# EndlessReform/smoltts

Measured on AMD Instinct MI355X. Metric: Mimi frames/sec (=12.5 x RTF), greedy DualAR decode + Mimi decode to PCM, higher is better.
Workload: dtype bf16 weights, fp32 activations/accumulate, fp32 KV cache (LM); fp32 (Mimi)

## Files before the change

include/smoltts_hip.h:

```cpp
#ifndef SMOLTTS_HIP_H
#define SMOLTTS_HIP_H

#include <stddef.h>
#include <stdint.h>

#ifdef __cplusplus
extern "C" {
#endif

#define SMOLTTS_ABI_VERSION 8

enum {
  SMOLTTS_OK = 0,
  SMOLTTS_E_INVALID = -1,
  SMOLTTS_E_HIP = -2,
  SMOLTTS_E_STATE = -3,
  SMOLTTS_E_CAPACITY = -4
};

const char* smoltts_last_error(void);
int smoltts_abi_version(void);



typedef struct SmolttsBlockWeights {
// ... 200 lines not shown

int smoltts_mimi_create(const SmolttsMimiConfig* cfg, const SmolttsMimiWeights* offsets,
                        const void* arena_dev, size_t arena_bytes, SmolttsMimi** out);
void smoltts_mimi_destroy(SmolttsMimi* m);

size_t smoltts_mimi_slab_bytes(const SmolttsMimi* m, int32_t max_batch, int32_t max_chunk_frames);
int smoltts_mimi_session_create(SmolttsMimi* m, void* slab_dev, size_t slab_bytes, int32_t max_batch,
                                int32_t max_chunk_frames, SmolttsMimiSession** out);
void smoltts_mimi_session_destroy(SmolttsMimiSession* s);
int smoltts_mimi_reset(SmolttsMimiSession* s, void* stream);

int smoltts_mimi_reset_slots(SmolttsMimiSession* s, const int32_t* slots_host, int32_t n_slots, void* stream);

#define SMOLTTS_MIMI_OPT_STATELESS_UPSAMPLE 1
#define SMOLTTS_MIMI_OPT_PRODUCTS 2
int smoltts_mimi_session_set_option(SmolttsMimiSession* s, int32_t option, int32_t value);

int smoltts_mimi_decode_chunk(SmolttsMimiSession* s, const int32_t* codes_dev, int64_t codes_stride,
                              int32_t frame_stride, int32_t code_offset, int32_t batch,
                              int32_t n_frames, float* pcm_dev, int64_t pcm_stride, void* stream);

typedef struct SmolttsMimiEncConfig {
  int32_t num_codebooks;
  int32_t n_layers;
  int32_t window;
  int32_t max_positions;
  int32_t extra_right;
} SmolttsMimiEncConfig;

typedef struct SmolttsMimiEncWeights {
// ... 323 lines not shown
                                   const SmolttsSlotFilters* filters_dev, const int32_t* frames_dev, const int32_t* history_dev,
                                   const int32_t* history_len_dev, int32_t step, int32_t* ids_dev, void* stream);

int smoltts_k_layernorm(const float* x_dev, const float* w_dev, const float* b_dev, int32_t n_rows,
                        int32_t dim, float eps, float* out_dev, void* stream);

int smoltts_k_seanet_resblock(int32_t channels, int32_t batch, int32_t n_rows, const float* x_dev, int64_t x_bstride,
                              const void* w2_w3_dev, const float* b2_dev, const void* w3_w3_dev, const float* b3_dev, float* out_dev,
                              int64_t o_bstride, int32_t b3_products, void* stream);

int smoltts_k_seanet_last(int32_t batch, int32_t n_rows, const float* in_dev, int64_t in_bstride, const void* wt_w3_dev,
                          const float* bt_dev, const void* w2_w3_dev, const float* b2_dev, const void* w3_w3_dev, const float* b3_dev,
                          const float* final_w_dev, float final_b, float* pcm_dev, int64_t pcm_stride, const int32_t* slot_pos_dev,
                          int32_t b3_products, void* stream);

int smoltts_k_rvq_upsample(const int32_t* codes_dev, int64_t codes_stride, int32_t frame_stride, int32_t code_offset, int32_t nq,
                           int32_t batch, int32_t n_frames, const float* table_dev, const float* upw_dev, const float* carry_in_dev,
                           float* carry_out_dev, float* tx_dev, void* stream);

#ifdef __cplusplus
}
#endif
#endif
```

smoltts_amd/abi.py:

```python
from __future__ import annotations

import ctypes as C
import os
import sys
from pathlib import Path
from typing import List, Optional

LIB_PATH = Path(__file__).resolve().parent / "csrc" / "libsmoltts_hip.so"


class SmolttsError(RuntimeError):
    pass


ABI_VERSION = 8
OK, E_INVALID, E_HIP, E_STATE, E_CAPACITY = 0, -1, -2, -3, -4
MAX_LAYERS, MAX_FAST_LAYERS, MIMI_MAX_LAYERS = 64, 16, 16
KV_F32, KV_BF16 = 0, 1
W_BF16, W_FP8 = 0, 1
OPT_QKV_TABLE, OPT_COMMIT_PICKS, OPT_SPLIT_ATTN, OPT_STREAM_W, OPT_FUSE_DEPTH_ATTN, OPT_FUSE_PICK, OPT_FP8_PREFILL = 1, 2, 3, 4, 5, 6, 7
MIMI_OPT_STATELESS_UPSAMPLE, MIMI_OPT_PRODUCTS = 1, 2
PRO_NONE, PRO_RMSNORM, PRO_ELU, PRO_LAYERNORM = 0, 1, 2, 3
EPI_STORE, EPI_RESID, EPI_SWIGLU, EPI_GELU, EPI_SCALE_RESID, EPI_QKV_ROPE = range(6)
RESAMPLE_OFF, RESAMPLE_S16, RESAMPLE_ULAW = 0, 1, 2
SEAM_FIRST, SEAM_FINAL, SEAM_OFF = 1, 2, 4
FLAC_OFF, FLAC_F32, FLAC_S16 = 0, 1, 2
FILTER_MAX_WINDOW, FILTER_MAX_PENALTY = 64, 1000.0
PREFIX_MAGIC, PREFIX_MAX_INSTALL = 0x58464250, 16

KV_FORMATS = {"fp32": KV_F32, "bf16": KV_BF16}


class BlockWeights(C.Structure):
    _fields_ = [(n, C.c_uint64) for n in ("attn_norm", "wqkv", "wo", "ffn_norm", "w13", "w2")]


# ... 210 lines not shown
    "smoltts_gemm3_attn_fusable": (INT, "i i i"),
    "smoltts_k_gemm3": (INT, "Gemm3Args* p"),
    "smoltts_k_x3_pack": (INT, "p q i i p p p p p p"),
    "smoltts_k_attention": (INT, "p p p p p i i i i i p p p"),
    "smoltts_k_attention_kv": (INT, "p p p p p i i i i i p p i p"),
    "smoltts_k_attention_split": (INT, "p p p p p i i i i i p p i p p p"),
    "smoltts_k_attention_rows3": (INT, "p p p p p i i i i i p i p"),
    "smoltts_k_embed": (INT, "p i i p p i i i i i i p p"),
    "smoltts_k_argmax": (INT, "p i i q p i p p"),
    "smoltts_k_sample": (INT, "p i i q f f Q i i p p"),
    "smoltts_k_sample_rows": (INT, "p i i q p p i p p"),
    "smoltts_k_sample_rows_filtered": (INT, "p i i q p p p p p i p p"),
    "smoltts_k_layernorm": (INT, "p p p i i f p p"),
    "smoltts_k_seanet_resblock": (INT, "i i i p q p p p p p q i p"),
    "smoltts_k_seanet_last": (INT, "i i p q p p p p p p p f p q p i p"),
    "smoltts_k_rvq_upsample": (INT, "p q i i i i i p p p p p p"),
}
DEBUG_HOOKS = {
    "smoltts_profile_begin": (INT, "i i i i"),
    "smoltts_profile_end": (INT, "f* i*"),
}


def _argtype(kind: str):
    if kind.endswith("*"):
        return C.POINTER(_KINDS.get(kind[:-1]) or globals()[kind[:-1]])
    return _KINDS[kind]


def _bind(lib, table) -> None:
# ... 40 lines not shown
```

smoltts_amd/build.py:

```python
from __future__ import annotations

import hashlib
import os
import shutil
import subprocess
import sys
from concurrent.futures import ThreadPoolExecutor
from pathlib import Path
from typing import Optional, Sequence

CSRC = Path(__file__).resolve().parent / "csrc"
LIB = CSRC / "libsmoltts_hip.so"
SOURCES = ["api.hip", "gemm.hip", "gemm_b3.hip", "gemm3.hip", "attention.hip", "small_ops.hip", "lm_engine.hip", "mimi_engine.hip", "mimi_encoder.hip",
           "seanet.hip", "seanet_last.hip", "conv_xs.hip", "conv_ks.hip", "resample.hip", "tsm.hip", "flac.hip", "seam.hip", "trim.hip", "loudness.hip",
           "watermark.hip"]
ARCH = "gfx950"
PRODUCT_FLAGS = [f"--offload-arch={ARCH}", "-O3", "-fPIC", "-std=c++17", "-Wno-unused-result", "-mllvm", "-amdgpu-kernarg-preload-count=16"]
NAMED_VARIANTS = {"hooks": ["-DSMOLTTS_DEBUG_HOOKS"],
                  "knobs": ["-DSMOLTTS_DBG_KNOBS"],
                  "lds_poison": ["-DSMOLTTS_DBG_LDS_POISON"]}


def _hipcc() -> str:
    for cand in (os.environ.get("HIPCC"), "/opt/rocm/bin/hipcc", shutil.which("hipcc")):
        if cand and Path(cand).exists():
            return cand
    raise RuntimeError("hipcc not found (looked at $HIPCC, /opt/rocm/bin/hipcc, PATH)")


# ... 68 lines not shown
```

smoltts_amd/csrc/api.hip:

```cpp
#include <stdarg.h>

#include "common.h"
#include "mimi_common.h"

namespace smoltts {
static thread_local char g_err[1024] = "";

void set_error(const char* fmt, ...) {
  va_list ap;
  va_start(ap, fmt);
  vsnprintf(g_err, sizeof(g_err), fmt, ap);
  va_end(ap);
}
}

using namespace smoltts;

extern "C" {

const char* smoltts_last_error(void) { return g_err; }
int smoltts_abi_version(void) { return SMOLTTS_ABI_VERSION; }

int smoltts_k_gemm(const SmolttsGemmArgs* a, void* stream) {
  ST_REQUIRE(a, SMOLTTS_E_INVALID, "k_gemm: null args");
// ... 93 lines not shown
                          const float* final_w_dev, float final_b, float* pcm_dev, int64_t pcm_stride, const int32_t* slot_pos_dev,
                          int32_t b3_products, void* stream) {
  ST_REQUIRE(pcm_stride >= 4 * (int64_t)n_rows, SMOLTTS_E_INVALID, "k_seanet_last: pcm_stride %lld < 4 * %d rows", (long long)pcm_stride,
             n_rows);
  MimiLastStageArgs a;
  memset(&a, 0, sizeof(a));
  a.batch = batch; a.T = n_rows;
  a.in = in_dev; a.in_bstride = in_bstride;
  a.wt = wt_w3_dev; a.bt = bt_dev; a.w2 = w2_w3_dev; a.b2 = b2_dev; a.w3 = w3_w3_dev; a.b3 = b3_dev;
  a.final_w = final_w_dev; a.final_b = final_b;
  a.pcm = pcm_dev; a.pcm_stride = pcm_stride;
  a.slot_pos = slot_pos_dev; a.b3_products = b3_products;
  return launch_seanet_last(a, (hipStream_t)stream);
}

int smoltts_k_rvq_upsample(const int32_t* codes_dev, int64_t codes_stride, int32_t frame_stride, int32_t code_offset, int32_t nq,
                           int32_t batch, int32_t n_frames, const float* table_dev, const float* upw_dev, const float* carry_in_dev,
                           float* carry_out_dev, float* tx_dev, void* stream) {
  return launch_rvq_upsample(codes_dev, codes_stride, frame_stride, code_offset, nq, batch, n_frames, table_dev, upw_dev, carry_in_dev,
                             carry_out_dev, tx_dev, (hipStream_t)stream);
}

}
```

smoltts_amd/csrc/mimi_common.h:

```cpp
#pragma once
#include "common.h"

namespace smoltts {

constexpr int MIMI_D = 512, MIMI_HEADS = 8, MIMI_FF = 2048;

struct MimiTransformerBufs {
  float *tx, *tn, *tq, *ta, *th;
  float *kc, *vc;
  size_t layer_stride;
  const int *row_pos, *row_slot;
  float* tws = nullptr;
  char *kc3 = nullptr, *vc3 = nullptr;
  size_t layer_stride3 = 0;
  int b3_products = 6;
};

int run_mimi_transformer(const char* arena, const SmolttsMimiLayerWeights* layers, int n_layers, const float* rope,
                         int cache_len, int window, const MimiTransformerBufs& b, int rows, int rows_per_slot,
                         float* last_out, int64_t last_bstride, hipStream_t st);

int launch_mimi_rows(int n_rows, int rows_per_slot, int pos0, int* row_pos, int* row_slot, hipStream_t st,
                     const int* slot_pos = nullptr);

// ... 8 lines not shown
int launch_seanet_resblock(const MimiResblockArgs& a, hipStream_t st);

struct MimiLastStageArgs {
  int batch, T;
  const float* in; int64_t in_bstride;
  const void* wt; const float* bt;
  const void* w2; const float* b2;
  const void* w3; const float* b3;
  const float* final_w; float final_b;
  float* pcm; int64_t pcm_stride;
  const int* slot_pos;
  int b3_products;
};
int launch_seanet_last(const MimiLastStageArgs& a, hipStream_t st);

int launch_rvq_upsample(const int* codes, int64_t codes_stride, int frame_stride, int code_offset, int nq, int batch, int n_frames,
                        const float* table, const float* upw, const float* carry_in, float* carry_out, float* tx, hipStream_t st);

inline SmolttsGemmArgs mimi_gemm_f32(const void* w, const float* x, long ldx, int M, int N, int K, const void* w3 = nullptr) {
  SmolttsGemmArgs a;
  memset(&a, 0, sizeof(a));
  a.w_dev = w; a.w_is_fp32 = 1; a.x_dev = x; a.ldx = ldx; a.M = M; a.N = N; a.K = K;
  a.w3_dev = w3;
  return a;
}

}
```

smoltts_amd/csrc/mimi_engine.hip:

```cpp
#include <stdlib.h>
#include <string.h>

#include <new>

#include "mimi_common.h"

using namespace smoltts;

namespace {
constexpr int D = MIMI_D, HEADS = MIMI_HEADS, FF = MIMI_FF, NCONV = 14, NBUF = 14;
constexpr int SAMPLES = 1920;
constexpr int BUF_C[NBUF] = {512, 1024, 512, 256, 512, 256, 128, 256, 128, 64, 128, 64, 32, 64};
constexpr int BUF_HALO[NBUF] = {6, 1, 2, 0, 1, 2, 0, 1, 2, 0, 2, 0, 0, 0};
constexpr bool FUSED_BLOCK[NCONV] = {false, false, false, false, false, false, false, false, true, false, false, false, false, false};
constexpr int LAST_STAGE = 10;
constexpr bool buf_used(int i) { return i <= LAST_STAGE && !(i >= 1 && FUSED_BLOCK[i - 1]); }
constexpr int BUF_RPF[NBUF] = {2, 2, 16, 16, 16, 96, 96, 96, 480, 480, 480, 1920, 1920, 1920};
}

struct SmolttsMimi {
  SmolttsMimiConfig cfg;
  SmolttsMimiWeights w;
  const char* arena;
  size_t arena_bytes;
};

struct SmolttsMimiSession {
  SmolttsMimi* m;
  int B, chunk;
  float* carry[2];
// ... 2 lines not shown
  float *kc, *vc;
  char *kc3, *vc3;
  size_t kv3_layer;
  int *row_pos, *row_slot;
  float* buf[NBUF];
  size_t buf_bstride[NBUF];
  size_t halo_total;
  char* zero_begin;
  size_t zero_bytes;
  int* pos_dev;
  float final_bias;
  int* pos_host;
  int parity;
  int products;
  int stateless_upsample;
};

namespace {

size_t carve(SmolttsMimiSession* s, char* base) {
  Carver cv{base, 0};
  const size_t B = s->B, F = s->chunk, R = B * 2 * F;
  const SmolttsMimiConfig& c = s->m->cfg;
  const size_t z0 = cv.off;
  s->carry[0] = cv.take<float>(B * D);
  s->carry[1] = cv.take<float>(B * D);
  s->pos_dev = cv.take<int>(B);
  for (int i = 0; i < NBUF; ++i) {
    s->buf_bstride[i] = buf_used(i) ? (size_t)(BUF_HALO[i] + BUF_RPF[i] * F) * BUF_C[i] : 0;
    s->buf[i] = cv.take<float>(B * s->buf_bstride[i]);
// ... 189 lines not shown
  tmp.B = max_batch; tmp.chunk = max_chunk_frames;
  return carve(&tmp, nullptr);
}

int smoltts_mimi_session_create(SmolttsMimi* m, void* slab_dev, size_t slab_bytes, int32_t max_batch,
                                int32_t max_chunk_frames, SmolttsMimiSession** out) {
  ST_REQUIRE(m && slab_dev && out && max_batch > 0 && max_chunk_frames > 0, SMOLTTS_E_INVALID, "mimi_session_create: bad argument");
  ST_REQUIRE(((uintptr_t)slab_dev & 255) == 0, SMOLTTS_E_INVALID, "mimi_session_create: slab must be 256-byte aligned");
  ST_REQUIRE(2 * max_chunk_frames <= m->cfg.max_positions, SMOLTTS_E_CAPACITY, "mimi_session_create: chunk exceeds max_positions");
  const size_t need = smoltts_mimi_slab_bytes(m, max_batch, max_chunk_frames);
  ST_REQUIRE(slab_bytes >= need, SMOLTTS_E_CAPACITY, "mimi_session_create: slab has %zu bytes, %zu needed", slab_bytes, need);
  SmolttsMimiSession* s = new (std::nothrow) SmolttsMimiSession;
  ST_REQUIRE(s, SMOLTTS_E_INVALID, "mimi_session_create: out of host memory");
  memset(s, 0, sizeof(*s));
  s->m = m; s->B = max_batch; s->chunk = max_chunk_frames;
  carve(s, (char*)slab_dev);
  s->pos_host = static_cast<int*>(calloc((size_t)max_batch, sizeof(int)));
  if (s->pos_host == nullptr || hipMemset(s->zero_begin, 0, s->zero_bytes) != hipSuccess ||
      (s->kc3 && (hipMemset(s->kc3, 0, s->kv3_layer * m->cfg.n_layers) != hipSuccess || hipMemset(s->vc3, 0, s->kv3_layer * m->cfg.n_layers) != hipSuccess)) ||
      hipMemcpy(&s->final_bias, m->arena + m->w.convs[NCONV - 1].b, sizeof(float), hipMemcpyDeviceToHost) != hipSuccess) {
    free(s->pos_host);
    delete s;
    set_error("mimi_session_create: allocation or hipMemset failed");
    return SMOLTTS_E_HIP;
  }
  *out = s;
  return SMOLTTS_OK;
}

void smoltts_mimi_session_destroy(SmolttsMimiSession* s) {
// ... 3 lines not shown
}

int smoltts_mimi_reset(SmolttsMimiSession* s, void* stream) {
  ST_REQUIRE(s, SMOLTTS_E_INVALID, "mimi_reset: null session");
  ST_CHECK_HIP(hipMemsetAsync(s->zero_begin, 0, s->zero_bytes, (hipStream_t)stream));
  for (int b = 0; b < s->B; ++b) s->pos_host[b] = 0;
  s->parity = 0;
  return SMOLTTS_OK;
}

int smoltts_mimi_session_set_option(SmolttsMimiSession* s, int32_t option, int32_t value) {
  ST_REQUIRE(s, SMOLTTS_E_INVALID, "mimi_session_set_option: null session");
  if (option == SMOLTTS_MIMI_OPT_PRODUCTS) {
    ST_REQUIRE(value == 3 || value == 6, SMOLTTS_E_INVALID, "mimi_session_set_option: products %d (3 or 6)", value);
    s->products = value;
    return SMOLTTS_OK;
  }
  ST_REQUIRE(option == SMOLTTS_MIMI_OPT_STATELESS_UPSAMPLE, SMOLTTS_E_INVALID, "mimi_session_set_option: unknown option %d", option);
  ST_REQUIRE(value == 0 || value == 1, SMOLTTS_E_INVALID, "mimi_session_set_option: value %d (0 or 1)", value);
  s->stateless_upsample = value;
  return SMOLTTS_OK;
}

int smoltts_mimi_reset_slots(SmolttsMimiSession* s, const int32_t* slots_host, int32_t n_slots, void* stream) {
  ST_REQUIRE(s && slots_host && n_slots > 0, SMOLTTS_E_INVALID, "mimi_reset_slots: bad argument");
  hipStream_t st = (hipStream_t)stream;
  for (int i = 0; i < n_slots; ++i) {
    const int b = slots_host[i];
    ST_TRY(check_slot("mimi_reset_slots", b, s->B));
    ST_CHECK_HIP(hipMemsetAsync(s->carry[0] + (size_t)b * D, 0, D * sizeof(float), st));
// ... 65 lines not shown
    if (i == LAST_STAGE) {
      const SmolttsMimiConv &c2 = m->w.convs[i + 1], &c3 = m->w.convs[i + 2];
      ST_REQUIRE(cv.w3 && c2.w3 && c3.w3 && m->w.final_w && cv.cin == 128 && cv.cout == 64 && cv.stride == 4, SMOLTTS_E_INVALID,
                 "mimi: the arena lacks the W3 tiles of the last stage (or its shape is not 128 -> 64, stride 4)");
      MimiLastStageArgs a;
      memset(&a, 0, sizeof(a));
      a.batch = batch; a.T = BUF_RPF[i] * F;
      a.in = s->buf[i] + (size_t)BUF_HALO[i] * BUF_C[i]; a.in_bstride = (int64_t)s->buf_bstride[i];
      a.wt = A + cv.w3; a.bt = (const float*)(A + cv.b);
      a.w2 = A + c2.w3; a.b2 = (const float*)(A + c2.b); a.w3 = A + c3.w3; a.b3 = (const float*)(A + c3.b);
      a.final_w = (const float*)(A + m->w.final_w); a.final_b = s->final_bias; a.pcm = pcm_dev; a.pcm_stride = pcm_stride;
      a.slot_pos = s->pos_dev; a.b3_products = s->products;
      ST_TRY(launch_seanet_last(a, st));
      break;
    }
    if (FUSED_BLOCK[i]) {
      const SmolttsMimiConv& c1 = m->w.convs[i + 1];
      ST_REQUIRE(cv.w3 && c1.w3, SMOLTTS_E_INVALID, "mimi: the arena lacks the W3 tiles of conv %d", i);
      MimiResblockArgs a;
      memset(&a, 0, sizeof(a));
      a.channels = cv.cin; a.batch = batch; a.T = BUF_RPF[i] * F;
      a.x = s->buf[i] + (size_t)BUF_HALO[i] * BUF_C[i]; a.x_bstride = (int64_t)s->buf_bstride[i];
      a.w2 = A + cv.w3; a.b2 = (const float*)(A + cv.b); a.w3 = A + c1.w3; a.b3 = (const float*)(A + c1.b);
      a.out = s->buf[i + 2] + (size_t)BUF_HALO[i + 2] * BUF_C[i + 2]; a.o_bstride = (int64_t)s->buf_bstride[i + 2];
      a.b3_products = s->products;
      ST_TRY(launch_seanet_resblock(a, st));
      i += 1;
      continue;
    }
    const int Tin = BUF_RPF[i] * F;
// ... 43 lines not shown
```

smoltts_amd/mimi.py:

```python
from __future__ import annotations

import ctypes as C
from typing import Dict, Optional, Sequence

import torch

from . import packing
from .abi import (MIMI_OPT_PRODUCTS, MIMI_OPT_STATELESS_UPSAMPLE, MimiConfig, MimiEncConfig, MimiEncLayout, MimiEncWeights, MimiWeights, SmolttsError, check,
                  load_library)
from .device import ClosesOnDel, _alloc_slab, _require_gpu, current_stream_ptr, dptr


class MimiEngine(ClosesOnDel):
    def __init__(self, state: Optional[Dict[str, torch.Tensor]], num_codebooks: int = 8, window: int = 0,
                 max_positions: int = 4096, arena: Optional[torch.Tensor] = None, offsets=None):
        self.lib = load_library()
        self.device = _require_gpu()
        if arena is None:
            arena, offsets = packing.pack_mimi(state, num_codebooks, max_positions)
        off = offsets
        max_positions = off["max_positions"]
        self.arena = arena.to(self.device)
        self.num_codebooks = num_codebooks
        cfg = MimiConfig(num_codebooks, off["n_layers"], window, max_positions)
# ... 101 lines not shown
        out["res"] = view(lay.res, lay.F, 256)
        out["dots"] = view(lay.dots, lay.F, 2048)
        return out

    def close(self):
        if getattr(self, "handle", None):
            self.lib.smoltts_mimi_encoder_destroy(self.handle)
            self.handle = None


class MimiSession(ClosesOnDel):

    SAMPLES_PER_FRAME = 1920
    OPT_STATELESS_UPSAMPLE = MIMI_OPT_STATELESS_UPSAMPLE
    OPT_PRODUCTS = MIMI_OPT_PRODUCTS

    def __init__(self, engine: MimiEngine, max_batch: int, max_chunk_frames: int = 8, stateless_upsample: bool = False,
                 products: int = 6):
        self.engine, self.lib = engine, engine.lib
        self.B, self.chunk = max_batch, max_chunk_frames
        need = self.lib.smoltts_mimi_slab_bytes(engine.handle, max_batch, max_chunk_frames)
        if need == 0:
            raise SmolttsError("smoltts_mimi_slab_bytes returned 0 (bad sizes)")
        self.slab = _alloc_slab(need, engine.device, settle=True)
        h = C.c_void_p()
        check(self.lib.smoltts_mimi_session_create(engine.handle, dptr(self.slab), need, max_batch, max_chunk_frames, C.byref(h)),
              "smoltts_mimi_session_create")
        self.handle = h
        if stateless_upsample:
            self.set_stateless_upsample(True)
        if products != 6:
            self.set_products(products)

    def set_products(self, n: int) -> None:
        check(self.lib.smoltts_mimi_session_set_option(self.handle, self.OPT_PRODUCTS, int(n)), "smoltts_mimi_session_set_option")

    def set_stateless_upsample(self, on: bool) -> None:
        check(self.lib.smoltts_mimi_session_set_option(self.handle, self.OPT_STATELESS_UPSAMPLE, int(bool(on))),
              "smoltts_mimi_session_set_option")

    def reset(self) -> None:
        check(self.lib.smoltts_mimi_reset(self.handle, current_stream_ptr()), "smoltts_mimi_reset")

    def reset_slots(self, slots: Sequence[int]) -> None:
        arr = (C.c_int32 * len(slots))(*slots)
        check(self.lib.smoltts_mimi_reset_slots(self.handle, arr, len(slots), current_stream_ptr()), "smoltts_mimi_reset_slots")

    def decode_chunk(self, codes: torch.Tensor, f0: int, n_frames: int, pcm: torch.Tensor, code_offset: int = 0) -> None:
        batch, F, row = codes.shape
        assert codes.dtype == torch.int32 and codes.is_contiguous() and pcm.dtype == torch.float32 and pcm.is_contiguous()
        assert batch <= self.B and n_frames <= self.chunk and f0 + n_frames <= F
# ... 20 lines not shown
```

smoltts_amd/ops.py:

```python
from __future__ import annotations

import ctypes as C
from dataclasses import dataclass
from typing import Optional

import torch

from . import abi as E
from .abi import Gemm3Args, PickArgs, SlotFilters, SlotSampling
from .device import current_stream_ptr, dptr
from .packing import tile_t16x32, tile_w3


def _k(name: str, *args) -> None:
    E.check(getattr(E.load_library(), name)(*args, current_stream_ptr()), name)


def pack_weight(w: torch.Tensor, fp32: bool = False) -> torch.Tensor:
    flat = tile_t16x32(w.detach().float().cpu(), torch.float32 if fp32 else torch.bfloat16)
    return flat.cuda()


def pack_weight_w3(w: torch.Tensor) -> torch.Tensor:
    return tile_w3(w.detach().float().cpu()).view(torch.uint8).cuda()
# ... 192 lines not shown
    return out


def seanet_last(inbuf: torch.Tensor, T: int, wt_w3: torch.Tensor, bt: torch.Tensor, w2_w3: torch.Tensor, b2: torch.Tensor,
                w3_w3: torch.Tensor, b3: torch.Tensor, final_w: torch.Tensor, final_b: float, slot_pos: torch.Tensor, pcm: torch.Tensor,
                b3_products: int = 6) -> torch.Tensor:
    S, rows, Cn = inbuf.shape
    assert inbuf.dtype == pcm.dtype == torch.float32 and Cn == 128 and inbuf.stride(2) == 1 and inbuf.stride(1) == Cn and pcm.stride(1) == 1
    assert pcm.shape[0] == S and 0 < T <= rows - 2 and 4 * T <= pcm.shape[1] and slot_pos.dtype == torch.int32 and slot_pos.numel() >= S
    assert bt.numel() == 256 and final_w.numel() == 192
    _k("smoltts_k_seanet_last", S, T, inbuf.data_ptr() + 4 * 2 * Cn, inbuf.stride(0), dptr(wt_w3), dptr(bt), dptr(w2_w3), dptr(b2),
       dptr(w3_w3), dptr(b3), dptr(final_w), float(final_b), dptr(pcm), pcm.stride(0), dptr(slot_pos), b3_products)
    return pcm


def rvq_upsample(codes: torch.Tensor, f0: int, n_frames: int, nq: int, table: torch.Tensor, upw: torch.Tensor,
                 carry_in: Optional[torch.Tensor], carry_out: torch.Tensor, code_offset: int = 0) -> torch.Tensor:
    S, F, row = codes.shape
    assert codes.dtype == torch.int32 and codes.is_contiguous() and 0 <= f0 and n_frames > 0 and f0 + n_frames <= F
    assert tuple(table.shape) == (nq, 2048, 512) and table.is_contiguous() and tuple(upw.shape) == (4, 512) and upw.is_contiguous()
    assert carry_out.numel() >= S * 512 and (carry_in is None or carry_in.numel() >= S * 512)
    tx = torch.empty(S, 2 * n_frames, 512, dtype=torch.float32, device=codes.device)
    _k("smoltts_k_rvq_upsample", codes.data_ptr() + 4 * f0 * row, F * row, row, code_offset, nq, S, n_frames, dptr(table), dptr(upw),
       dptr(carry_in), dptr(carry_out), dptr(tx))
    return tx


def x3_bytes(rows: int, K: int) -> int:
    return (rows + 15) // 16 * 16 * K * 6

# ... 90 lines not shown
```

Before: 28470.

## Fuse SEANet stage 3 transposed conv and residual block into one kernel

Adds a kernel that runs the stride-5 transposed conv (256->128) together with the following residual block (k3 conv to 64, k1 conv back to 128, skip add, ELU) in one launch. Intermediates stay in LDS as split bf16 pieces, and the carry tail rows are written out for streaming. It is on by default, with a session option to turn it off. The aim is to cut two kernel launches and the global-memory round trips of the upsampled intermediate, at the cost of a complex hand-scheduled kernel that uses a lot of LDS and may run at lower occupancy.

```diff
diff --git a/include/smoltts_hip.h b/include/smoltts_hip.h
--- a/include/smoltts_hip.h
+++ b/include/smoltts_hip.h
@@ -8,7 +8,7 @@
 extern "C" {
 #endif
 
-#define SMOLTTS_ABI_VERSION 8
+#define SMOLTTS_ABI_VERSION 9
 
 enum {
   SMOLTTS_OK = 0,
@@ -239,6 +239,7 @@
 
 #define SMOLTTS_MIMI_OPT_STATELESS_UPSAMPLE 1
 #define SMOLTTS_MIMI_OPT_PRODUCTS 2
+#define SMOLTTS_MIMI_OPT_FUSE_STAGE3 3
 int smoltts_mimi_session_set_option(SmolttsMimiSession* s, int32_t option, int32_t value);
 
 int smoltts_mimi_decode_chunk(SmolttsMimiSession* s, const int32_t* codes_dev, int64_t codes_stride,
@@ -592,6 +593,11 @@
                           const float* final_w_dev, float final_b, float* pcm_dev, int64_t pcm_stride, const int32_t* slot_pos_dev,
                           int32_t b3_products, void* stream);
 
+int smoltts_k_seanet_stage3(int32_t batch, int32_t n_rows, const float* in_dev, int64_t in_bstride, const void* wt_w3_dev,
+                            const float* bt_dev, const void* w2_w3_dev, const float* b2_dev, const void* w3_w3_dev, const float* b3_dev,
+                            float* out_dev, int64_t o_bstride, float* tail_dev, int64_t tail_bstride, const int32_t* slot_pos_dev,
+                            int32_t b3_products, void* stream);
+
 int smoltts_k_rvq_upsample(const int32_t* codes_dev, int64_t codes_stride, int32_t frame_stride, int32_t code_offset, int32_t nq,
                            int32_t batch, int32_t n_frames, const float* table_dev, const float* upw_dev, const float* carry_in_dev,
                            float* carry_out_dev, float* tx_dev, void* stream);
diff --git a/smoltts_amd/abi.py b/smoltts_amd/abi.py
--- a/smoltts_amd/abi.py
+++ b/smoltts_amd/abi.py
@@ -13,13 +13,13 @@
     pass
 
 
-ABI_VERSION = 8
+ABI_VERSION = 9
 OK, E_INVALID, E_HIP, E_STATE, E_CAPACITY = 0, -1, -2, -3, -4
 MAX_LAYERS, MAX_FAST_LAYERS, MIMI_MAX_LAYERS = 64, 16, 16
 KV_F32, KV_BF16 = 0, 1
 W_BF16, W_FP8 = 0, 1
 OPT_QKV_TABLE, OPT_COMMIT_PICKS, OPT_SPLIT_ATTN, OPT_STREAM_W, OPT_FUSE_DEPTH_ATTN, OPT_FUSE_PICK, OPT_FP8_PREFILL = 1, 2, 3, 4, 5, 6, 7
-MIMI_OPT_STATELESS_UPSAMPLE, MIMI_OPT_PRODUCTS = 1, 2
+MIMI_OPT_STATELESS_UPSAMPLE, MIMI_OPT_PRODUCTS, MIMI_OPT_FUSE_STAGE3 = 1, 2, 3
 PRO_NONE, PRO_RMSNORM, PRO_ELU, PRO_LAYERNORM = 0, 1, 2, 3
 EPI_STORE, EPI_RESID, EPI_SWIGLU, EPI_GELU, EPI_SCALE_RESID, EPI_QKV_ROPE = range(6)
 RESAMPLE_OFF, RESAMPLE_S16, RESAMPLE_ULAW = 0, 1, 2
@@ -260,6 +260,7 @@
     "smoltts_k_layernorm": (INT, "p p p i i f p p"),
     "smoltts_k_seanet_resblock": (INT, "i i i p q p p p p p q i p"),
     "smoltts_k_seanet_last": (INT, "i i p q p p p p p p p f p q p i p"),
+    "smoltts_k_seanet_stage3": (INT, "i i p q p p p p p p p q p q p i p"),
     "smoltts_k_rvq_upsample": (INT, "p q i i i i i p p p p p p"),
 }
 DEBUG_HOOKS = {
diff --git a/smoltts_amd/build.py b/smoltts_amd/build.py
--- a/smoltts_amd/build.py
+++ b/smoltts_amd/build.py
@@ -12,7 +12,7 @@
 CSRC = Path(__file__).resolve().parent / "csrc"
 LIB = CSRC / "libsmoltts_hip.so"
 SOURCES = ["api.hip", "gemm.hip", "gemm_b3.hip", "gemm3.hip", "attention.hip", "small_ops.hip", "lm_engine.hip", "mimi_engine.hip", "mimi_encoder.hip",
-           "seanet.hip", "seanet_last.hip", "conv_xs.hip", "conv_ks.hip", "resample.hip", "tsm.hip", "flac.hip", "seam.hip", "trim.hip", "loudness.hip",
+           "seanet.hip", "seanet_stage.hip", "seanet_last.hip", "conv_xs.hip", "conv_ks.hip", "resample.hip", "tsm.hip", "flac.hip", "seam.hip", "trim.hip", "loudness.hip",
            "watermark.hip"]
 ARCH = "gfx950"
 PRODUCT_FLAGS = [f"--offload-arch={ARCH}", "-O3", "-fPIC", "-std=c++17", "-Wno-unused-result", "-mllvm", "-amdgpu-kernarg-preload-count=16"]
diff --git a/smoltts_amd/csrc/api.hip b/smoltts_amd/csrc/api.hip
--- a/smoltts_amd/csrc/api.hip
+++ b/smoltts_amd/csrc/api.hip
@@ -131,6 +131,20 @@
   return launch_seanet_last(a, (hipStream_t)stream);
 }
 
+int smoltts_k_seanet_stage3(int32_t batch, int32_t n_rows, const float* in_dev, int64_t in_bstride, const void* wt_w3_dev,
+                            const float* bt_dev, const void* w2_w3_dev, const float* b2_dev, const void* w3_w3_dev, const float* b3_dev,
+                            float* out_dev, int64_t o_bstride, float* tail_dev, int64_t tail_bstride, const int32_t* slot_pos_dev,
+                            int32_t b3_products, void* stream) {
+  MimiStage3Args a;
+  memset(&a, 0, sizeof(a));
+  a.batch = batch; a.T = n_rows;
+  a.in = in_dev; a.in_bstride = in_bstride;
+  a.wt = wt_w3_dev; a.bt = bt_dev; a.w2 = w2_w3_dev; a.b2 = b2_dev; a.w3 = w3_w3_dev; a.b3 = b3_dev;
+  a.out = out_dev; a.o_bstride = o_bstride; a.tail = tail_dev; a.tail_bstride = tail_bstride;
+  a.slot_pos = slot_pos_dev; a.b3_products = b3_products;
+  return launch_seanet_stage3(a, (hipStream_t)stream);
+}
+
 int smoltts_k_rvq_upsample(const int32_t* codes_dev, int64_t codes_stride, int32_t frame_stride, int32_t code_offset, int32_t nq,
                            int32_t batch, int32_t n_frames, const float* table_dev, const float* upw_dev, const float* carry_in_dev,
                            float* carry_out_dev, float* tx_dev, void* stream) {
diff --git a/smoltts_amd/csrc/mimi_common.h b/smoltts_amd/csrc/mimi_common.h
--- a/smoltts_amd/csrc/mimi_common.h
+++ b/smoltts_amd/csrc/mimi_common.h
@@ -46,6 +46,19 @@
 };
 int launch_seanet_last(const MimiLastStageArgs& a, hipStream_t st);
 
+struct MimiStage3Args {
+  int batch, T;
+  const float* in; int64_t in_bstride;
+  const void* wt; const float* bt;
+  const void* w2; const float* b2;
+  const void* w3; const float* b3;
+  float* out; int64_t o_bstride;
+  float* tail; int64_t tail_bstride;
+  const int* slot_pos;
+  int b3_products;
+};
+int launch_seanet_stage3(const MimiStage3Args& a, hipStream_t st);
+
 int launch_rvq_upsample(const int* codes, int64_t codes_stride, int frame_stride, int code_offset, int nq, int batch, int n_frames,
                         const float* table, const float* upw, const float* carry_in, float* carry_out, float* tx, hipStream_t st);
 
diff --git a/smoltts_amd/csrc/mimi_engine.hip b/smoltts_amd/csrc/mimi_engine.hip
--- a/smoltts_amd/csrc/mimi_engine.hip
+++ b/smoltts_amd/csrc/mimi_engine.hip
@@ -11,9 +11,10 @@
 constexpr int D = MIMI_D, HEADS = MIMI_HEADS, FF = MIMI_FF, NCONV = 14, NBUF = 14;
 constexpr int SAMPLES = 1920;
 constexpr int BUF_C[NBUF] = {512, 1024, 512, 256, 512, 256, 128, 256, 128, 64, 128, 64, 32, 64};
-constexpr int BUF_HALO[NBUF] = {6, 1, 2, 0, 1, 2, 0, 1, 2, 0, 2, 0, 0, 0};
+constexpr int BUF_HALO[NBUF] = {6, 1, 2, 0, 1, 2, 0, 2, 2, 0, 2, 0, 0, 0};
 constexpr bool FUSED_BLOCK[NCONV] = {false, false, false, false, false, false, false, false, true, false, false, false, false, false};
 constexpr int LAST_STAGE = 10;
+constexpr int STAGE3 = 7;
 constexpr bool buf_used(int i) { return i <= LAST_STAGE && !(i >= 1 && FUSED_BLOCK[i - 1]); }
 constexpr int BUF_RPF[NBUF] = {2, 2, 16, 16, 16, 96, 96, 96, 480, 480, 480, 1920, 1920, 1920};
 }
@@ -46,6 +47,7 @@
   int parity;
   int products;
   int stateless_upsample;
+  int fuse_stage3;
 };
 
 namespace {
@@ -265,6 +267,7 @@
   ST_REQUIRE(s, SMOLTTS_E_INVALID, "mimi_session_create: out of host memory");
   memset(s, 0, sizeof(*s));
   s->m = m; s->B = max_batch; s->chunk = max_chunk_frames;
+  s->fuse_stage3 = 1;
   carve(s, (char*)slab_dev);
   s->pos_host = static_cast<int*>(calloc((size_t)max_batch, sizeof(int)));
   if (s->pos_host == nullptr || hipMemset(s->zero_begin, 0, s->zero_bytes) != hipSuccess ||
@@ -298,6 +301,11 @@
   if (option == SMOLTTS_MIMI_OPT_PRODUCTS) {
     ST_REQUIRE(value == 3 || value == 6, SMOLTTS_E_INVALID, "mimi_session_set_option: products %d (3 or 6)", value);
     s->products = value;
+    return SMOLTTS_OK;
+  }
+  if (option == SMOLTTS_MIMI_OPT_FUSE_STAGE3) {
+    ST_REQUIRE(value == 0 || value == 1, SMOLTTS_E_INVALID, "mimi_session_set_option: value %d (0 or 1)", value);
+    s->fuse_stage3 = value;
     return SMOLTTS_OK;
   }
   ST_REQUIRE(option == SMOLTTS_MIMI_OPT_STATELESS_UPSAMPLE, SMOLTTS_E_INVALID, "mimi_session_set_option: unknown option %d", option);
@@ -393,6 +401,22 @@
       ST_TRY(launch_seanet_last(a, st));
       break;
     }
+    if (i == STAGE3 && s->fuse_stage3 && cv.w3 && m->w.convs[i + 1].w3 && m->w.convs[i + 2].w3 && cv.transposed && cv.cin == 256 &&
+        cv.cout == 128 && cv.stride == 5) {
+      const SmolttsMimiConv &c2 = m->w.convs[i + 1], &c3 = m->w.convs[i + 2];
+      MimiStage3Args a;
+      memset(&a, 0, sizeof(a));
+      a.batch = batch; a.T = BUF_RPF[i] * F;
+      a.in = s->buf[i] + (size_t)BUF_HALO[i] * BUF_C[i]; a.in_bstride = (int64_t)s->buf_bstride[i];
+      a.wt = A + cv.w3; a.bt = (const float*)(A + cv.b);
+      a.w2 = A + c2.w3; a.b2 = (const float*)(A + c2.b); a.w3 = A + c3.w3; a.b3 = (const float*)(A + c3.b);
+      a.out = s->buf[i + 3] + (size_t)BUF_HALO[i + 3] * BUF_C[i + 3]; a.o_bstride = (int64_t)s->buf_bstride[i + 3];
+      a.tail = s->buf[i + 1] + (size_t)BUF_RPF[i + 1] * F * BUF_C[i + 1]; a.tail_bstride = (int64_t)s->buf_bstride[i + 1];
+      a.slot_pos = s->pos_dev; a.b3_products = s->products;
+      ST_TRY(launch_seanet_stage3(a, st));
+      i += 2;
+      continue;
+    }
     if (FUSED_BLOCK[i]) {
       const SmolttsMimiConv& c1 = m->w.convs[i + 1];
       ST_REQUIRE(cv.w3 && c1.w3, SMOLTTS_E_INVALID, "mimi: the arena lacks the W3 tiles of conv %d", i);
diff --git a/smoltts_amd/csrc/seanet_stage.hip b/smoltts_amd/csrc/seanet_stage.hip
--- /dev/null
+++ b/smoltts_amd/csrc/seanet_stage.hip
@@ -0,0 +1,373 @@
+#include "gemm_dev.h"
+#include "mimi_common.h"
+
+namespace smoltts {
+
+namespace {
+
+struct StageDev {
+  const float* in;
+  long in_bstride;
+  int T;
+  const char* wt;
+  const float* bt;
+  const char* w2;
+  const float* b2;
+  const char* w3;
+  const float* b3;
+  float* out;
+  long o_bstride;
+  float* tail;
+  long tail_bstride;
+  const int* slot_pos;
+  int tiles_per_slot, n_tiles, tiles_per_wg;
+};
+
+__device__ __forceinline__ float elu_st(float x) { return x > 0.f ? x : __expf(x) - 1.0f; }
+
+constexpr int CI = 256, C = 128, H = 64, J = 5;
+constexpr int S = 64, MT = S / 16;
+constexpr int RA = (S + 2 + 15) / 16 * 16;
+constexpr int PL = 19, PR = 96;
+constexpr int RC = J * 16;
+constexpr int KA = 2 * CI / 32, K2 = 3 * C / 32, K3 = H / 32;
+constexpr int AP_U4 = 3 * (CI / 8) * RA, HP_U4 = 3 * (C / 8) * PR, VP_U4 = 3 * (H / 8) * RC;
+constexpr int REGION_U4 = AP_U4 > HP_U4 + VP_U4 ? AP_U4 : HP_U4 + VP_U4;
+constexpr int STASH_U4 = 8 * 4 * 2;
+constexpr int BIAS_U4 = (H + C) / 4;
+constexpr size_t LDS_BYTES = (size_t)(REGION_U4 + STASH_U4 + BIAS_U4) * 16;
+constexpr int IN_IT = ((S + 2 + 7) / 8 * 8 * (CI / 8) + 511) / 512;
+#ifdef SMOLTTS_DBG_ST3_AHEAD
+constexpr int WB_AHEAD = SMOLTTS_DBG_ST3_AHEAD;
+#else
+constexpr int WB_AHEAD = 1;
+#endif
+static_assert(J * PL <= PR && PL >= 17 && RA >= S + 2 && WB_AHEAD >= 1 && WB_AHEAD <= 3, "plane sizes");
+
+template <int NP>
+__global__ __launch_bounds__(512) void seanet_stage3_kernel(StageDev p) {
+  extern __shared__ __attribute__((aligned(16))) char smem[];
+  uint4* ap = reinterpret_cast<uint4*>(smem);
+  uint4* hp = reinterpret_cast<uint4*>(smem);
+  uint4* vp = hp + HP_U4;
+  f32x4* stash = reinterpret_cast<f32x4*>(smem) + REGION_U4;
+  float* bias_l = reinterpret_cast<float*>(stash + STASH_U4);
+  const int tid0 = threadIdx.x;
+  const int wave = __builtin_amdgcn_readfirstlane(tid0 >> 6);
+#define ST_LANE_IDS                                                                                                     \
+  int tid = tid0;                                                                                                       \
+  asm volatile("" : "+v"(tid));                                                                                         \
+  const int lane = tid & 63, r = lane & 15, q = lane >> 4, wlane = lane * 16;
+  const int ctb = __builtin_amdgcn_readfirstlane(wave & 3), pb0 = __builtin_amdgcn_readfirstlane(wave >> 2);
+
+  const char* w2tile = p.w2 + (size_t)ctb * K2 * 3072;
+  const char* w3tile = p.w3 + (size_t)wave * K3 * 3072;
+
+#define ST_FETCH_ROWS(TILE)                                                                                              \
+  {                                                                                                                     \
+    const int fb_ = (TILE) / p.tiles_per_slot, fs0_ = ((TILE) - fb_ * p.tiles_per_slot) * S;                            \
+    const float* src_ = p.in + (long)fb_ * p.in_bstride;                                                                \
+    _Pragma("unroll") for (int it_ = 0; it_ < IN_IT; ++it_) {                                                           \
+      const int idx_ = tid + 512 * it_, i_ = (idx_ >> 8) * 8 + (idx_ & 7), g8_ = (idx_ >> 3) & 31, row_ = fs0_ - 2 + i_; \
+      const bool on_ = (TILE) < t_end && i_ <= S + 1 && row_ < p.T;        \
+      pre[it_][0] = on_ ? *reinterpret_cast<const float4*>(src_ + (long)row_ * CI + g8_ * 8) : make_float4(0.f, 0.f, 0.f, 0.f);     \
+      pre[it_][1] = on_ ? *reinterpret_cast<const float4*>(src_ + (long)row_ * CI + g8_ * 8 + 4) : make_float4(0.f, 0.f, 0.f, 0.f); \
+    }                                                                                                                   \
+  }
+  const int t_begin = (int)blockIdx.x * p.tiles_per_wg;
+  const int t_end = t_begin + p.tiles_per_wg < p.n_tiles ? t_begin + p.tiles_per_wg : p.n_tiles;
+#define ST_STORE_ROWS                                                                                                   \
+  _Pragma("unroll") for (int it = 0; it < IN_IT; ++it) {                                                                \
+    const int idx = tid + 512 * it, i = (idx >> 8) * 8 + (idx & 7), g8 = (idx >> 3) & 31;                               \
+    if (i > S + 1) continue;                                                                                            \
+    uint4 h, m, l;                                                                                                      \
+    split3x8(pre[it][0], pre[it][1], h, m, l);                                                                          \
+    const int slot = g8 * RA + i;                         \
+    ap[slot] = h;                                                                                                       \
+    ap[slot + (CI / 8) * RA] = m;                                                                                       \
+    ap[slot + 2 * (CI / 8) * RA] = l;                                                                                   \
+  }
+  if (tid0 < H + C) bias_l[tid0] = tid0 < H ? p.b2[tid0] : p.b3[tid0 - H];
+  if (t_begin < t_end) {
+    const int tid = tid0;
+    float4 pre[IN_IT][2];
+    ST_FETCH_ROWS(t_begin)
+    ST_STORE_ROWS
+  }
+
+#define ST_PIECES(V, PROW)                                                                                              \
+  {                                                                                                                     \
+    uint32_t h0, m0, l0, h1, m1, l1;                                                                                    \
+    split3_pair((V)[0], (V)[1], h0, m0, l0);                                                                            \
+    split3_pair((V)[2], (V)[3], h1, m1, l1);                                                                            \
+    const int s2 = ((((wave >> 1) * 4) + (wave & 1) * 2 + (q >> 1)) * PR + (PROW)) * 2 + (q & 1);  \
+    hp2[s2] = make_uint2(h0, h1);                                                                                       \
+    hp2[s2 + (C / 8) * PR * 2] = make_uint2(m0, m1);                                                                    \
+    hp2[s2 + 2 * (C / 8) * PR * 2] = make_uint2(l0, l1);                                                                \
+  }
+#define ST_PHASE0(Q)                                                                                                    \
+  _Pragma("unroll") for (int j = 0; j < J; ++j) {                                                                       \
+    const f32x4 v = acc[Q][j];                                                                                          \
+    const float e[4] = {elu_st(v[0]), elu_st(v[1]), elu_st(v[2]), elu_st(v[3])};                                        \
+    ST_PIECES(e, j * PL + r + 1)                                                                                        \
+  }                                                                                                                     \
+  if (r == 15) {                                                                                                        \
+    _Pragma("unroll") for (int j = J - 2; j < J; ++j) {                                                                 \
+      f32x4 v;                                                                                                          \
+      if ((Q) > 0) v = acc[(Q) > 0 ? (Q) - 1 : 0][j]; else v = stash[(wave * 4 + q) * 2 + j - (J - 2)];                 \
+      const bool pad = (Q) == 0 && stream_start;                                                                        \
+      const float e[4] = {pad ? 0.f : elu_st(v[0]), pad ? 0.f : elu_st(v[1]), pad ? 0.f : elu_st(v[2]), pad ? 0.f : elu_st(v[3])}; \
+      ST_PIECES(e, j * PL)                                                                                              \
+    }                                                                                                                   \
+  }
+#define ST_LOAD_W(DST, BASE, KC)                                                                                        \
+  _Pragma("unroll") for (int pc = 0; pc < 3; ++pc) (DST)[pc] = *reinterpret_cast<const uint4*>((BASE) + (size_t)(KC) * 3072 + pc * 1024 + wlane);
+
+  for (int tile = t_begin; tile < t_end; ++tile) {
+  const int b = tile / p.tiles_per_slot;
+  const int ti = tile - b * p.tiles_per_slot;
+  const int s0 = ti * S;
+  const bool stream_start = ti == 0 && p.slot_pos[b] == 0;
+  const bool need_halo = !stream_start && (tile == t_begin || ti == 0);
+
+  f32x4 acc[MT][J];
+  {
+  ST_LANE_IDS
+  lds_barrier();
+
+#pragma unroll
+  for (int mt = 0; mt < MT; ++mt)
+#pragma unroll
+    for (int j = 0; j < J; ++j) acc[mt][j] = (f32x4){0.f, 0.f, 0.f, 0.f};
+  {
+    const char* wtile = p.wt + (size_t)wave * KA * 3072;
+    uint4 wq[2][J][3];
+#ifndef SMOLTTS_DBG_ST3_NO_A
+    if (need_halo) {
+      f32x4 ha[2] = {(f32x4){0.f, 0.f, 0.f, 0.f}, (f32x4){0.f, 0.f, 0.f, 0.f}};
+      uint4 wh[4][2][3];
+#pragma unroll
+      for (int kc = 0; kc < 3; ++kc)
+#pragma unroll
+        for (int jj = 0; jj < 2; ++jj) ST_LOAD_W(wh[kc][jj], wtile, (J - 2 + jj) * 8 * KA + kc)
+#pragma unroll
+      for (int kc = 0; kc < KA; ++kc) {
+        if (kc + 3 < KA) {
+#pragma unroll
+          for (int jj = 0; jj < 2; ++jj) ST_LOAD_W(wh[(kc + 3) & 3][jj], wtile, (J - 2 + jj) * 8 * KA + kc + 3)
+        }
+        __builtin_amdgcn_sched_barrier(0);
+        uint4 xf[3];
+#pragma unroll
+        for (int pc = 0; pc < 3; ++pc) xf[pc] = ap[((pc * 8 + (kc & 7)) * 4 + q) * RA + r + (kc >> 3)];
+#pragma unroll
+        for (int jj = 0; jj < 2; ++jj) ha[jj] = mfma_b3<NP>(wh[kc & 3][jj], xf, ha[jj]);
+      }
+      if (r == 0) {
+#pragma unroll
+        for (int jj = 0; jj < 2; ++jj) {
+          const float4 bb = *reinterpret_cast<const float4*>(p.bt + ((J - 2 + jj) * 8 + wave) * 16 + 4 * q);
+          f32x4 v = ha[jj];
+          v[0] += bb.x; v[1] += bb.y; v[2] += bb.z; v[3] += bb.w;
+          stash[(wave * 4 + q) * 2 + jj] = v;
+        }
+      }
+    }
+#endif
+#pragma unroll
+    for (int j = 0; j < J; ++j) ST_LOAD_W(wq[0][j], wtile, j * 8 * KA)
+#ifndef SMOLTTS_DBG_ST3_NO_A
+    int tap = 0, xc = 0;
+#define ST_CHUNK(BUF, KC)                                                                                               \
+  {                                                                                                                     \
+    if ((KC) + 1 < KA) {                                                                                                \
+      _Pragma("unroll") for (int j = 0; j < J; ++j) ST_LOAD_W(wq[(BUF) ^ 1][j], wtile, j * 8 * KA + (KC) + 1)           \
+    }                                                                                                                   \
+    __builtin_amdgcn_sched_barrier(0);                                         \
+    _Pragma("unroll") for (int mt = 0; mt < MT; ++mt) {                                                                 \
+      uint4 xf[3];                                                                                                      \
+      _Pragma("unroll") for (int pc = 0; pc < 3; ++pc) xf[pc] = ap[((pc * 8 + xc) * 4 + q) * RA + mt * 16 + r + tap + 1]; \
+      _Pragma("unroll") for (int j = 0; j < J; ++j) acc[mt][j] = mfma_b3<NP>(wq[BUF][j], xf, acc[mt][j]);               \
+    }                                                                                                                   \
+    if (++xc == 8) { xc = 0; ++tap; }                                                                                   \
+  }
+#pragma unroll 1
+    for (int kc = 0; kc < KA; kc += 2) {
+      if ((wave >> 2) != 0) __builtin_amdgcn_s_setprio(1); else __builtin_amdgcn_s_setprio(0);
+      ST_CHUNK(0, kc)
+      if ((wave >> 2) == 0) __builtin_amdgcn_s_setprio(1); else __builtin_amdgcn_s_setprio(0);
+      ST_CHUNK(1, kc + 1)
+    }
+#undef ST_CHUNK
+#endif
+    __builtin_amdgcn_s_setprio(0);
+#pragma unroll
+    for (int j = 0; j < J; ++j) {
+      const float4 bb = *reinterpret_cast<const float4*>(p.bt + (j * 8 + wave) * 16 + 4 * q);
+#pragma unroll
+      for (int mt = 0; mt < MT; ++mt) {
+        acc[mt][j][0] += bb.x; acc[mt][j][1] += bb.y; acc[mt][j][2] += bb.z; acc[mt][j][3] += bb.w;
+      }
+    }
+  }
+  }
+  lds_barrier();
+  ST_LANE_IDS
+  int pb = pb0;
+  asm volatile("" : "+s"(pb));
+  float4 pre[IN_IT][2];
+  uint4 wb[4][3];
+#pragma unroll
+  for (int kc = 0; kc < WB_AHEAD; ++kc) ST_LOAD_W(wb[kc], w2tile, kc)
+
+  uint2* hp2 = reinterpret_cast<uint2*>(hp);
+  uint2* vp2 = reinterpret_cast<uint2*>(vp);
+
+#ifdef SMOLTTS_DBG_ST3_NO_QUARTERS
+  if (acc[0][0][0] == 12345.f) {
+    float sum = 0.f;
+    for (int mt = 0; mt < MT; ++mt)
+      for (int j = 0; j < J; ++j) sum += acc[mt][j][0] + acc[mt][j][1] + acc[mt][j][2] + acc[mt][j][3];
+    p.out[tid] = sum;
+  }
+  lds_barrier();
+#else
+  ST_PHASE0(0)
+  lds_barrier();
+#pragma unroll
+  for (int Q = 0; Q < MT; ++Q) {
+    int wl_o = wlane;
+    asm volatile("" : "+v"(wl_o));
+    const int wlane = wl_o;
+    if (Q == MT - 1) {
+      int tid_s = tid;
+      asm volatile("" : "+v"(tid_s));
+      const int tid = tid_s;
+      ST_FETCH_ROWS(tile + 1)
+    }
+    uint4 w3r[K3][3];
+    {
+      f32x4 hb[3] = {(f32x4){0.f, 0.f, 0.f, 0.f}, (f32x4){0.f, 0.f, 0.f, 0.f}, (f32x4){0.f, 0.f, 0.f, 0.f}};
+#pragma unroll
+      for (int kc = 0; kc < K2; ++kc) {
+        if (kc + WB_AHEAD < K2) ST_LOAD_W(wb[(kc + WB_AHEAD) & 3], w2tile, kc + WB_AHEAD)
+        __builtin_amdgcn_sched_barrier(0);
+        const int d = kc >> 2, xc = kc & 3;
+#pragma unroll
+        for (int i = 0; i < 3; ++i) {
+          if (i == 2 && wave >= 4) continue;
+          const int jp = i == 2 ? 4 : pb + 2 * i;
+          const int jj = jp - 2 + d;
+          const int prow = (jj < 0 ? jj + J : jj) * PL + r + (jj < 0 ? 0 : 1);
+          uint4 xf[3];
+#pragma unroll
+          for (int pc = 0; pc < 3; ++pc) xf[pc] = hp[((pc * 4 + xc) * 4 + q) * PR + prow];
+          hb[i] = mfma_b3<NP>(wb[kc & 3], xf, hb[i]);
+        }
+      }
+#pragma unroll
+      for (int kc = 0; kc < K3; ++kc) ST_LOAD_W(w3r[kc], w3tile, kc)
+      const float4 b2_r = *reinterpret_cast<const float4*>(bias_l + ctb * 16 + 4 * q);
+#pragma unroll
+      for (int i = 0; i < 3; ++i) {
+        if (i == 2 && wave >= 4) continue;
+        const int jp = i == 2 ? 4 : pb + 2 * i;
+        const int row = jp * 16 + r;
+        const float v0 = elu_st(hb[i][0] + b2_r.x), v1 = elu_st(hb[i][1] + b2_r.y), v2 = elu_st(hb[i][2] + b2_r.z), v3 = elu_st(hb[i][3] + b2_r.w);
+        uint32_t h0, m0, l0, h1, m1, l1;
+        split3_pair(v0, v1, h0, m0, l0);
+        split3_pair(v2, v3, h1, m1, l1);
+        const int s2 = (((ctb >> 1) * 4 + (ctb & 1) * 2 + (q >> 1)) * RC + row) * 2 + (q & 1);
+        vp2[s2] = make_uint2(h0, h1);
+        vp2[s2 + (H / 8) * RC * 2] = make_uint2(m0, m1);
+        vp2[s2 + 2 * (H / 8) * RC * 2] = make_uint2(l0, l1);
+      }
+    }
+    lds_barrier();
+
+    {
+      f32x4 y[J];
+#pragma unroll
+      for (int j = 0; j < J; ++j) {
+        y[j] = (f32x4){0.f, 0.f, 0.f, 0.f};
+#pragma unroll
+        for (int kc = 0; kc < K3; ++kc) {
+          uint4 xf[3];
+#pragma unroll
+          for (int pc = 0; pc < 3; ++pc) xf[pc] = vp[((pc * K3 + kc) * 4 + q) * RC + j * 16 + r];
+          y[j] = mfma_b3<NP>(w3r[kc], xf, y[j]);
+        }
+      }
+      if (Q + 1 < MT) {
+#pragma unroll
+        for (int kc = 0; kc < WB_AHEAD; ++kc) ST_LOAD_W(wb[kc], w2tile, kc)
+        ST_PHASE0(Q + 1)
+      }
+      if (Q + 1 == MT && r == 15) {
+#pragma unroll
+        for (int j = J - 2; j < J; ++j) stash[(wave * 4 + q) * 2 + j - (J - 2)] = acc[Q][j];
+      }
+      int r_o = r;
+      asm volatile("" : "+v"(r_o));
+      const int srow = s0 + Q * 16 + r_o;
+      const bool live = srow < p.T;
+      if (live) {
+        const float4 b3_r = *reinterpret_cast<const float4*>(bias_l + H + wave * 16 + 4 * q);
+        float* orow = p.out + (long)b * p.o_bstride + (long)srow * (J * C) + wave * 16 + 4 * q;
+#pragma unroll
+        for (int j = 0; j < J; ++j) {
+          const f32x4 x = acc[Q][j];
+          *reinterpret_cast<float4*>(orow + j * C) = make_float4(elu_st(y[j][0] + b3_r.x + x[0]), elu_st(y[j][1] + b3_r.y + x[1]),
+                                                                 elu_st(y[j][2] + b3_r.z + x[2]), elu_st(y[j][3] + b3_r.w + x[3]));
+        }
+        if (p.tail != nullptr && srow == p.T - 1) {
+          float* trow = p.tail + (long)b * p.tail_bstride + wave * 16 + 4 * q;
+#pragma unroll
+          for (int j = J - 2; j < J; ++j)
+            *reinterpret_cast<float4*>(trow + (j - (J - 2)) * C) = make_float4(acc[Q][j][0], acc[Q][j][1], acc[Q][j][2], acc[Q][j][3]);
+        }
+      }
+    }
+    lds_barrier();
+  }
+  ST_STORE_ROWS
+#endif
+  }
+#undef ST_LANE_IDS
+#undef ST_FETCH_ROWS
+#undef ST_STORE_ROWS
+#undef ST_PHASE0
+#undef ST_PIECES
+#undef ST_LOAD_W
+}
+
+}
+
+int launch_seanet_stage3(const MimiStage3Args& a, hipStream_t st) {
+  ST_REQUIRE(a.in && a.wt && a.bt && a.w2 && a.b2 && a.w3 && a.b3 && a.out && a.slot_pos && a.T > 0 && a.batch > 0, SMOLTTS_E_INVALID,
+             "seanet stage 3: null or empty argument");
+  ST_REQUIRE(a.batch <= 65535, SMOLTTS_E_INVALID, "seanet stage 3: batch too large");
+  ST_REQUIRE(a.in_bstride % 4 == 0 && a.o_bstride % 4 == 0 && a.tail_bstride % 4 == 0 && ((uintptr_t)a.in & 15) == 0 && ((uintptr_t)a.out & 15) == 0 &&
+                 ((uintptr_t)a.tail & 15) == 0,
+             SMOLTTS_E_INVALID, "seanet stage 3: rows must be 16-byte aligned");
+  static PerDevice attr;
+  const int dev = PerDevice::current();
+  if (!attr.done(dev)) {
+    ST_CHECK_HIP(hipFuncSetAttribute((const void*)seanet_stage3_kernel<6>, hipFuncAttributeMaxDynamicSharedMemorySize, (int)LDS_BYTES));
+    ST_CHECK_HIP(hipFuncSetAttribute((const void*)seanet_stage3_kernel<3>, hipFuncAttributeMaxDynamicSharedMemorySize, (int)LDS_BYTES));
+    attr.mark_done(dev);
+  }
+  const int tiles_per_slot = (a.T + S - 1) / S;
+  ST_REQUIRE((long)tiles_per_slot * a.batch < (1L << 30), SMOLTTS_E_INVALID, "seanet stage 3: too many rows for one launch");
+  StageDev d{a.in, (long)a.in_bstride, a.T, (const char*)a.wt, a.bt, (const char*)a.w2, a.b2, (const char*)a.w3, a.b3,
+             a.out, (long)a.o_bstride, a.tail, (long)a.tail_bstride, a.slot_pos, tiles_per_slot, tiles_per_slot * a.batch, 0};
+  const int n_cu = device_cu_count(), g0 = d.n_tiles < n_cu ? d.n_tiles : n_cu;
+  d.tiles_per_wg = (d.n_tiles + g0 - 1) / g0;
+  const dim3 grid((d.n_tiles + d.tiles_per_wg - 1) / d.tiles_per_wg);
+  if (a.b3_products == 3) hipLaunchKernelGGL(seanet_stage3_kernel<3>, grid, dim3(512), LDS_BYTES, st, d);
+  else hipLaunchKernelGGL(seanet_stage3_kernel<6>, grid, dim3(512), LDS_BYTES, st, d);
+  ST_CHECK_HIP(hipGetLastError());
+  return SMOLTTS_OK;
+}
+
+}
diff --git a/smoltts_amd/mimi.py b/smoltts_amd/mimi.py
--- a/smoltts_amd/mimi.py
+++ b/smoltts_amd/mimi.py
@@ -6,7 +6,7 @@
 import torch
 
 from . import packing
-from .abi import (MIMI_OPT_PRODUCTS, MIMI_OPT_STATELESS_UPSAMPLE, MimiConfig, MimiEncConfig, MimiEncLayout, MimiEncWeights, MimiWeights, SmolttsError, check,
+from .abi import (MIMI_OPT_FUSE_STAGE3, MIMI_OPT_PRODUCTS, MIMI_OPT_STATELESS_UPSAMPLE, MimiConfig, MimiEncConfig, MimiEncLayout, MimiEncWeights, MimiWeights, SmolttsError, check,
                   load_library)
 from .device import ClosesOnDel, _alloc_slab, _require_gpu, current_stream_ptr, dptr
 
@@ -139,6 +139,7 @@
     SAMPLES_PER_FRAME = 1920
     OPT_STATELESS_UPSAMPLE = MIMI_OPT_STATELESS_UPSAMPLE
     OPT_PRODUCTS = MIMI_OPT_PRODUCTS
+    OPT_FUSE_STAGE3 = MIMI_OPT_FUSE_STAGE3
 
     def __init__(self, engine: MimiEngine, max_batch: int, max_chunk_frames: int = 8, stateless_upsample: bool = False,
                  products: int = 6):
@@ -160,6 +161,9 @@
     def set_products(self, n: int) -> None:
         check(self.lib.smoltts_mimi_session_set_option(self.handle, self.OPT_PRODUCTS, int(n)), "smoltts_mimi_session_set_option")
 
+    def set_fuse_stage3(self, on: bool) -> None:
+        check(self.lib.smoltts_mimi_session_set_option(self.handle, self.OPT_FUSE_STAGE3, int(bool(on))), "smoltts_mimi_session_set_option")
+
     def set_stateless_upsample(self, on: bool) -> None:
         check(self.lib.smoltts_mimi_session_set_option(self.handle, self.OPT_STATELESS_UPSAMPLE, int(bool(on))),
               "smoltts_mimi_session_set_option")
diff --git a/smoltts_amd/ops.py b/smoltts_amd/ops.py
--- a/smoltts_amd/ops.py
+++ b/smoltts_amd/ops.py
@@ -230,6 +230,22 @@
     return pcm
 
 
+def seanet_stage3(inbuf: torch.Tensor, T: int, wt_w3: torch.Tensor, bt: torch.Tensor, w2_w3: torch.Tensor, b2: torch.Tensor,
+                  w3_w3: torch.Tensor, b3: torch.Tensor, slot_pos: torch.Tensor, out: torch.Tensor, out_lead: int = 0,
+                  tail: Optional[torch.Tensor] = None, b3_products: int = 6) -> torch.Tensor:
+    S, rows, Cn = inbuf.shape
+    assert inbuf.dtype == out.dtype == torch.float32 and Cn == 256 and inbuf.stride(2) == 1 and inbuf.stride(1) == Cn
+    assert out.shape[0] == S and out.shape[2] == 128 and out.stride(2) == 1 and out.stride(1) == 128
+    assert 0 < T <= rows - 2 and out_lead + 5 * T <= out.shape[1] and slot_pos.dtype == torch.int32 and slot_pos.numel() >= S
+    assert bt.numel() == 640
+    if tail is not None:
+        assert tail.dtype == torch.float32 and tail.shape == (S, 2, 128) and tail.stride(2) == 1 and tail.stride(1) == 128
+    _k("smoltts_k_seanet_stage3", S, T, inbuf.data_ptr() + 4 * 2 * Cn, inbuf.stride(0), dptr(wt_w3), dptr(bt), dptr(w2_w3), dptr(b2),
+       dptr(w3_w3), dptr(b3), out.data_ptr() + 4 * out_lead * 128, out.stride(0), dptr(tail), tail.stride(0) if tail is not None else 0,
+       dptr(slot_pos), b3_products)
+    return out
+
+
 def rvq_upsample(codes: torch.Tensor, f0: int, n_frames: int, nq: int, table: torch.Tensor, upw: torch.Tensor,
                  carry_in: Optional[torch.Tensor], carry_out: torch.Tensor, code_offset: int = 0) -> torch.Tensor:
     S, F, row = codes.shape
```

After: 28610 (median of 6 runs). About the same (+0.5%).
